# ajyoon/rocoder

Measured on AMD Instinct MI355X. Metric: output Msamples/s, 16384-win f=8 stereo (x CPU-realtime in config), higher is better.
Workload: dtype f32

## Files before the change

rocoder_amd/csrc/rc_hop16k.hip:

```cpp
#include "rc_dit.hpp"

namespace rc {
namespace {

constexpr int f1_idx(int n) { return n + (n >> 5); }
constexpr int HOP2_XBUF = 8192 + 256 + 32;
constexpr int HOP2_LDS_FLOAT2 = HOP2_XBUF + 8 + 32 + 256 + 256 + 16 + 24 + 1024;
constexpr int F3_W[13] = {1, 2, 4, 8, 16, 32, 64, 131, 259, 520, 1038, 2079, 4156};
constexpr int f3_idx(int n) {
    int r = 0;
    for (int i = 0; i < 13; ++i) r += ((n >> i) & 1) * F3_W[i];
    return r;
}

__global__ __launch_bounds__(256, 2) void hop2_kernel(const HopParams p) {
    constexpr int LOG2N = 14, m = 13, M = 1 << m, H = M, T = 256, P = 32, PH = 16;
    constexpr int RES = 512;
    constexpr int SCR = HOP2_XBUF + 8;
    constexpr int T_A = SCR + 32;
    constexpr int T_R = T_A + 256;
    constexpr int T_B = T_R + 256;
    constexpr int T_C = T_B + 16;
    constexpr int T_H = T_C + 24;
    static_assert(T_H + 1024 == HOP2_LDS_FLOAT2, "LDS layout");
    extern __shared__ __attribute__((aligned(16))) float2 lds[];
    const int tid = threadIdx.x;
    const uint32_t run = blockIdx.x % p.runs_per_channel;
    const uint32_t ch = blockIdx.x / p.runs_per_channel;
    const int64_t k_begin = p.hop_first + (int64_t)run * p.run_len;
    int64_t k_end = k_begin + p.run_len;
    if (k_end > p.hop_first + p.hop_count) k_end = p.hop_first + p.hop_count;
    if (k_begin >= k_end) return;
    GF xc = (GF)p.x + (size_t)ch * p.in_stride;
    GF xt = (GF)p.xtail + (size_t)ch * p.tail_stride;
    GFW outc = (GFW)p.out + (size_t)ch * p.out_stride;
    const unsigned lane2 = 2u * (unsigned)tid;
    GV2 wtab = (GV2)p.wtab;
    const uint32_t pitch = p.pitch;

    const int r = tid, rb = tid ? RES - tid : RES / 2;
    const int l4 = tid & 15, uu = tid >> 4;
    const int pos4 = (uu << 9) | l4;
    const int bE1s = f3_idx(((int)(__brev((unsigned)tid) >> 24) << 5));
    const int b4f3 = f3_idx(pos4);
    const int bAr = f3_idx(r), bBr = f3_idx(rb);
    const int bE3a = f3_idx(((int)(__brev((unsigned)r) >> 23) << 4));
    const int bE3b = f3_idx(((int)(__brev((unsigned)rb) >> 23) << 4));
    const int bE4l = f3_idx(tid);

    Stamps st;
    st.init();
    v2f tail[PH];
#pragma unroll
    for (int q = 0; q < PH; ++q) tail[q] = v2f{0.f, 0.f};

    {
        lds[T_A + tid] = ldg2(wtab + tid);
        lds[T_R + tid] = ldg2((GV2)p.rtab + tid);
        if (tid < 16) lds[T_B + tid] = ldg2(wtab + 16 * tid);
        if (tid <= 16) lds[T_C + tid] = ldg2(wtab + 128 * tid);
        __syncthreads();
    }
    float xr0[P], xr1[P];
    auto issue_x = [&](int64_t kk) {
        GF src = hop_src(p, xc, xt, kk);
#pragma unroll
        for (int q = 0; q < P; ++q) {
            xr0[q] = (src + 2 * T * q)[lane2];
            xr1[q] = (src + 2 * T * q)[lane2 + 1];
        }
    };
    auto win_f1 = [&](v2f (&vn)[P]) {
        GF win = per_hop(p.window);
        float wr0[P], wr1[P];
#pragma unroll
        for (int q = 0; q < P; ++q) {
            wr0[q] = (win + 2 * T * q)[lane2];
            wr1[q] = (win + 2 * T * q)[lane2 + 1];
        }
        __builtin_amdgcn_sched_barrier(0);
#pragma unroll
        for (int q = 0; q < P; ++q) vn[brev_c(q, 5)] = v2f{xr0[q], xr1[q]} * v2f{wr0[q], wr1[q]};
        __builtin_amdgcn_sched_barrier(0);
        st.mark(0);
        dit_stages<32, m, 0, 4, 0, false, false>(vn);
        st.mark(1);
    };
    auto epilogue = [&](int64_t kk, v2f (&ve)[P]) {
        GF wsrc = per_hop(p.window);
        float wr0[P], wr1[P];
#pragma unroll
        for (int q = 0; q < P; ++q) {
            wr0[q] = (wsrc + 2 * T * q)[lane2];
            wr1[q] = (wsrc + 2 * T * q)[lane2 + 1];
        }
        __builtin_amdgcn_sched_barrier(0);
#pragma unroll
        for (int q = 0; q < P; ++q) ve[q] *= v2f{wr0[q], wr1[q]};
        __builtin_amdgcn_sched_barrier(0);
        if (kk >= k_begin) {
            const int64_t g0 = kk * (int64_t)H;
            GF esrc = per_hop(p.env);
            const int64_t kq = g0 / pitch;
            const uint32_t kr = (uint32_t)(g0 % pitch);
            GFW dst = outc + (kq - p.out_origin);
            int t2 = tid;
            opaque(t2);
#pragma unroll
            for (int q = 0; q < PH; ++q) {
                const uint32_t i0 = 2u * (uint32_t)(t2 + T * q);
                const v2f er = v2f{(esrc + 2 * T * q)[lane2], (esrc + 2 * T * q)[lane2 + 1]};
                const v2f o = (ve[q] + tail[q]) * er * v2f{p.amp, p.amp};
                const float o0 = o.x, o1 = o.y;
                const uint32_t a0 = kr + i0, a1 = a0 + 1;
                const uint32_t d0 = a0 / pitch, d1 = a1 / pitch;
                if (d0 * pitch == a0) dst[d0] = o0;
                if (d1 * pitch == a1) dst[d1] = o1;
            }
        }
#pragma unroll
        for (int q = 0; q < PH; ++q) tail[q] = ve[q + PH];
        st.mark(21);
    };
    const int64_t k_first = k_begin > 0 ? k_begin - 1 : k_begin;
    v2f vn[P];
    for (int64_t k = k_first; k < k_end; ++k) {
        const PhaseKey key = make_phase_key(p.seed_mixed, p.ch_first + ch, k);
        v2f v[P];
        issue_x(k);
        win_f1(vn);
#pragma unroll
        for (int q = 0; q < P; ++q) lds[bE1s + f3_idx(q)] = to_f2(vn[q]);
        st.mark(2);
        __syncthreads();
        st.mark(3);
#pragma unroll
        for (int q = 0; q < P; ++q) v[q] = xld(lds, b4f3 + f3_idx(q << 4));
        dit_stages<32, m, 5, 8, 4, false, true>(v, to_v(lds[T_B + l4]));
        st.mark(4);
#pragma unroll
        for (int q = 0; q < P; ++q) lds[b4f3 + f3_idx(q << 4)] = to_f2(v[q]);
        st.mark(5);
        __syncthreads();
        st.mark(6);
        v2f va[16], vb[16];
#pragma unroll
        for (int q = 0; q < 16; ++q) {
            va[q] = xld(lds, bAr + f3_idx((RES * q)));
            vb[q] = xld(lds, bBr + f3_idx((RES * q)));
        }
        st.mark(7);
        __syncthreads();
        st.mark(8);
        {
            const v2f wa = to_v(lds[T_A + tid]);
            const v2f k16 = {W32_RE[2], W32_IM[2]};
            v2f wb = vcmul(v2f{wa.x, -wa.y}, k16);
            if (tid == 0) wb = v2f{W32_RE[1], W32_IM[1]};
            dit_stages<16, m, 9, 12, 9, false, true>(va, wa);
            dit_stages<16, m, 9, 12, 9, false, true>(vb, wb);
        }
        st.mark(9);

        if (tid == 0) {
#pragma unroll
            for (int q = 0; q < 16; ++q) {
                lds[SCR + q] = to_f2(va[q]);
                lds[SCR + 16 + q] = to_f2(vb[q]);
            }
        }
        {
            const int rr = r;
            const float2 wr = lds[T_R + tid];
            const uint32_t x0 = (uint32_t)rr * key.mul + key.k0;
            const uint32_t dx = (uint32_t)RES * key.mul;
#pragma unroll
            for (int q = 0; q < 16; ++q) {
                const v2f wrv = to_v(wr);
                const v2f wq = q == 0 ? wrv : (q == 8 ? v2f{wr.y, -wr.x}
                               : vcmul(wrv, v2f{W32_RE[q & 15], W32_IM[q & 15]}));
                v2f VA, VB;
                pair_regs_pk<LOG2N>(va[q], vb[15 - q], wq, x0 + (uint32_t)q * dx, key, VA, VB);
                va[q] = VA;
                vb[15 - q] = VB;
            }
        }
        st.mark(10);
        if (tid < 64) {
            const int i = tid;
            if (i <= 16) {
                int ja, ia, ib;
                if (i == 0) { ja = 0; ia = 0; ib = 0; }
                else if (i <= 7) { ja = RES * i; ia = i; ib = 16 - i; }
                else if (i == 8) { ja = RES * 8; ia = 8; ib = 8; }
                else { ja = RES / 2 + RES * (i - 9); ia = 16 + (i - 9); ib = 16 + 15 - (i - 9); }
                const float2 A = lds[SCR + ia], Bp = lds[SCR + ib];
                const float2 w = lds[T_C + (ja >> 8)];
                float2 VA, VB;
                pair_regs<LOG2N>(A, Bp, w, (uint32_t)ja * key.mul + key.k0, key, VA, VB, ja == 0);
                lds[SCR + ia] = VA;
                if (ib != ia) lds[SCR + ib] = VB;
            }
            if (tid == 0) {
#pragma unroll
                for (int q = 0; q < 16; ++q) {
                    va[q] = to_v(lds[SCR + q]);
                    vb[q] = to_v(lds[SCR + 16 + q]);
                }
            }
        }
        st.mark(11);
        v2f pa[16], pb[16];
#pragma unroll
        for (int q = 0; q < 16; ++q) {
            pa[brev_c(q, 4)] = va[q];
            pb[brev_c(q, 4)] = vb[q];
        }
        dit_stages<16, m, 0, 3, 0, true, false>(pa);
        dit_stages<16, m, 0, 3, 0, true, false>(pb);
        st.mark(12);
#pragma unroll
        for (int q = 0; q < 16; ++q) {
            lds[bE3a + f3_idx(q)] = to_f2(pa[q]);
            lds[bE3b + f3_idx(q)] = to_f2(pb[q]);
        }
        st.mark(13);
        __syncthreads();
        st.mark(14);
#pragma unroll
        for (int q = 0; q < P; ++q) v[q] = xld(lds, b4f3 + f3_idx(q << 4));
        dit_stages<32, m, 4, 8, 4, true, true>(v, to_v(lds[T_B + l4]));
        st.mark(15);
#pragma unroll
        for (int q = 0; q < P; ++q) lds[b4f3 + f3_idx(q << 4)] = to_f2(v[q]);
        st.mark(16);
        __syncthreads();
        st.mark(17);
#pragma unroll
        for (int q = 0; q < P; ++q) v[q] = xld(lds, bE4l + f3_idx((q << 8)));
        st.mark(18);
        __syncthreads();
        st.mark(19);
        dit_stages<32, m, 9, 12, 8, true, true>(v, to_v(lds[T_A + tid]));
        st.mark(20);

        epilogue(k, v);
    }
#if RC_STAMP
    if ((tid & 63) == 0 && p.spec) {
        unsigned *dbg = (unsigned *)p.spec + ((size_t)blockIdx.x * (T / 64) + (tid >> 6)) * 32;
        for (int i = 0; i < 32; ++i) dbg[i] = st.acc[i];
    }
#endif
}


constexpr int HOP4_REG = 1040;
constexpr int HOP4_XBUF = 4 * HOP4_REG;
constexpr int HOP4_LDS_FLOAT2 = HOP4_XBUF + 8 + 32 + 256 + 256 + 16 + 24 + 1024;
constexpr int phi_c(int l) { return (l & 1) ? 1 + 2 * (((l >> 1) ^ (l >> 2)) & 1) : 2 * ((l >> 1) & 1); }
constexpr int cidx_c(int l) { return (((l >> 2) & 1) << 1) | ((l >> 3) & 1); }
__device__ __forceinline__ void wave_fence() {
    __builtin_amdgcn_fence(__ATOMIC_RELEASE, "wavefront");
    asm volatile("" ::: "memory");
    __builtin_amdgcn_fence(__ATOMIC_ACQUIRE, "wavefront");
}

#define HOP4_BAR()                                                                    \
    do {                                                                              \
        asm volatile("s_waitcnt lgkmcnt(0)\n\ts_barrier" ::: "memory");                \
    } while (0)
__device__ __forceinline__ float band_gain(const HopParams &p, uint32_t f) {
    return (f - p.band_lo) <= p.band_span ? p.band_gin : p.band_gout;
}
template <int PITCHC, bool BAND = false, bool TABW = false>
__global__ __launch_bounds__(256, 3) void hop4_kernel(const HopParams p) {
    constexpr bool PITCH1 = PITCHC == 1;
    static_assert(!TABW || (PITCH1 && !BAND), "the table-window instantiation exists for pitch 1 without the band mask");
    constexpr int LOG2N = 14, m = 13, M = 1 << m, H = M, T = 256, P = 32, PH = 16;
    constexpr int RES = 512, REG = HOP4_REG;
    constexpr int SCR = HOP4_XBUF + 8;
    constexpr int T_A = SCR + 32;
    constexpr int T_R = T_A + 256;
    constexpr int T_B = T_R + 256;
    constexpr int T_C = T_B + 16;
    constexpr int T_H = T_C + 24;
    static_assert(T_H + 1024 == HOP4_LDS_FLOAT2, "LDS layout");
    extern __shared__ __attribute__((aligned(16))) float2 lds[];
    const int tid = threadIdx.x;
    uint32_t gr = blockIdx.x;
    const bool seam = p.seam_head != nullptr;
    if (seam) {
        unsigned *slot = reinterpret_cast<unsigned *>(lds + SCR);
        if (tid == 0) {
            const uint32_t total = p.runs_per_channel * p.n_channels;
            unsigned got = 0xFFFFFFFFu;
            {
                const uint32_t G = (total + 7u) / 8u;
                unsigned xcc;
                asm volatile("s_getreg_b32 %0, hwreg(HW_REG_XCC_ID)" : "=s"(xcc));
                for (uint32_t i = 0; i < 8u; ++i) {
                    const uint32_t xx = (xcc + i) & 7u, lo = xx * G;
                    if (lo >= total) continue;
                    const uint32_t hi = lo + G < total ? lo + G : total;
                    const uint32_t t = atomicAdd(p.run_counter + xx, 1u);
                    if (t < hi - lo) {
                        got = lo + t;
                        break;
                    }
                }
            }
            *slot = got;
        }
        __syncthreads();
        gr = (uint32_t)__builtin_amdgcn_readfirstlane((int)*reinterpret_cast<volatile unsigned *>(slot));
        __syncthreads();
        if (gr == 0xFFFFFFFFu) return;
    }
    const uint32_t run = gr % p.runs_per_channel;
    const uint32_t ch = gr / p.runs_per_channel;
    const int64_t k_begin = p.hop_first + (int64_t)run * p.run_len;
    int64_t k_end = k_begin + p.run_len;
    if (k_end > p.hop_first + p.hop_count) k_end = p.hop_first + p.hop_count;
    if (k_begin >= k_end) return;
    const bool stash_first = seam && run > 0;
    const bool has_next = seam && run + 1 < p.runs_per_channel;
    GF xc = (GF)p.x + (size_t)ch * p.in_stride;
    GF xt = (GF)p.xtail + (size_t)ch * p.tail_stride;
    GFW outc = (GFW)p.out + (size_t)ch * p.out_stride;
    const unsigned lane2 = 2u * (unsigned)tid;
    GV2 wtab = (GV2)p.wtab;
    const uint32_t pitch = PITCHC ? (uint32_t)PITCHC : p.pitch;

    struct Who {
        int wv, lane, cc, lo4, nib, r, A0;
    };
    int nib_keep, a0_keep;
    {
        const int w_ = tid >> 6, c_ = (tid >> 4) & 3;
        const int nl3 = c_ & 1, nl2 = c_ >> 1, nl0 = w_ & 1;
        const int nl1 = nl0 ? ((w_ >> 1) ^ nl2) : (w_ >> 1);
        nib_keep = (nl3 << 3) | (nl2 << 2) | (nl1 << 1) | nl0;
        a0_keep = w_ * REG + (tid & 63);
    }
    auto who = [&]() {
        int t = tid;
        opaque(t);
        Who w;
        w.wv = t >> 6;
        w.lane = t & 63;
        w.cc = (t >> 4) & 3;
        w.lo4 = t & 15;
        w.nib = nib_keep;
        w.r = (w.lo4 << 4) | w.nib;
        w.A0 = a0_keep;
        return w;
    };
    const int wv = tid >> 6;
    Stamps st;
    st.init();
    v2f tail[PH];
#pragma unroll
    for (int q = 0; q < PH; ++q) tail[q] = v2f{0.f, 0.f};
    {
        lds[T_A + tid] = ldg2(wtab + tid);
        lds[T_R + tid] = ldg2((GV2)p.rtab + tid);
        if (tid < 16) lds[T_B + tid] = ldg2(wtab + 16 * tid);
        if (tid <= 16) lds[T_C + tid] = ldg2(wtab + 128 * tid);
        if (tid == 0) {
            const float2 w256 = ldg2((GV2)p.rtab + 256);
            lds[SCR + 2] = make_float2(-w256.y, w256.x);
        }
        if constexpr (!TABW) {
#pragma unroll
            for (int i = 0; i < 2; ++i) {
                const float2 a = ldg2((GV2)p.hann_rot + 512 * i + 2 * tid);
                const float2 b = ldg2((GV2)p.hann_rot + 512 * i + 2 * tid + 1);
                lds[T_H + 512 * i + 2 * tid] = make_float2(a.x, b.x);
                lds[T_H + 512 * i + 2 * tid + 1] = make_float2(a.y, b.y);
            }
        }
        __syncthreads();
    }
    const v2f half2 = {0.5f, 0.5f};
    auto store_head = [&](int64_t kk, const auto &head) {
        const v2f amp2 = {p.amp, p.amp};
        const v2f cbE = to_v(lds[T_H + 2 * T + 2 * tid]) * amp2, sbE = to_v(lds[T_H + 2 * T + 2 * tid + 1]) * amp2;
        const v2f halfa = half2 * amp2;
        const int64_t g0 = kk * (int64_t)H;
        if constexpr (PITCH1) {
            const unsigned long long da = (unsigned long long)(outc + (g0 - p.out_origin));
            const unsigned dlo = __builtin_amdgcn_readfirstlane((unsigned)da);
            const unsigned dhi = __builtin_amdgcn_readfirstlane((unsigned)(da >> 32));
            GFW dst = (GFW)(((unsigned long long)dhi << 32) | dlo);
            const __amdgpu_buffer_rsrc_t rd = __builtin_amdgcn_make_buffer_rsrc((void *)dst, 0, 0x40000000, 0x00020000);
            typedef unsigned v2u __attribute__((ext_vector_type(2)));
#define HOP4_STORE(o, row)                                                                                                  \
    do {                                                                                                                    \
        if constexpr (!TABW)                                                                             \
            __builtin_amdgcn_raw_buffer_store_b64(v2u{__float_as_uint((o).x), __float_as_uint((o).y)}, rd,                 \
                                                  (int)(4u * lane2), 4 * 2 * T * (row), 2);                                 \
        else __builtin_nontemporal_store(o, (GV2W)(dst + 2 * T * (row) + lane2));                                           \
    } while (0)
            if constexpr (TABW) {
                GF et2 = per_hop(p.env) + lane2;
#pragma unroll
                for (int q0 = 0; q0 < PH; q0 += 4) {
                    float e0[4], e1[4];
#pragma unroll
                    for (int q = 0; q < 4; ++q) {
                        e0[q] = (et2 + 2 * T * (q0 + q))[0];
                        e1[q] = (et2 + 2 * T * (q0 + q))[1];
                    }
#pragma unroll
                    for (int q = 0; q < 4; ++q) {
                        const v2f o = (head[q0 + q] + tail[q0 + q]) * v2f{e0[q], e1[q]} * amp2;
                        HOP4_STORE(o, q0 + q);
                    }
                    __builtin_amdgcn_sched_barrier(0);
                }
                return;
            }
#pragma unroll
            for (int q = 0; q < PH; ++q) {
                const v2f er = __builtin_elementwise_fma(v2f{HANN_E14.s[q], HANN_E14.s[q]}, sbE,
                               __builtin_elementwise_fma(v2f{HANN_E14.c[q], HANN_E14.c[q]}, cbE, halfa));
                const v2f o = (head[q] + tail[q]) * er;
                HOP4_STORE(o, q);
            }
        } else {
            const int64_t kq = g0 / pitch;
            const uint32_t kr = (uint32_t)(g0 % pitch);
            GFW dst = outc + (kq - p.out_origin);
            int t2 = tid;
            opaque(t2);
            const unsigned long long da = (unsigned long long)dst;
            const unsigned dlo = __builtin_amdgcn_readfirstlane((unsigned)da);
            const unsigned dhi = __builtin_amdgcn_readfirstlane((unsigned)(da >> 32));
            const __amdgpu_buffer_rsrc_t rsrc = __builtin_amdgcn_make_buffer_rsrc(
                (void *)(((unsigned long long)dhi << 32) | dlo), 0, 0x40000000, 0x00020000);
            if constexpr (PITCHC > 1) {
                const PitchOffsets<PITCHC> po = pitch_offsets<PITCHC>(kr + 2u * (uint32_t)t2);
#pragma unroll
                for (int q = 0; q < PH; ++q) {
                    const v2f er = __builtin_elementwise_fma(v2f{HANN_E14.s[q], HANN_E14.s[q]}, sbE,
                                   __builtin_elementwise_fma(v2f{HANN_E14.c[q], HANN_E14.c[q]}, cbE, halfa));
                    const v2f o = (head[q] + tail[q]) * er;
                    const float ox = o.x, oy = o.y;
                    pitch_store_pair<PITCHC, 2 * T>(rsrc, po, q, ox, oy);
                }
                return;
            }
            constexpr uint32_t DROP = 0xFFFFFFFCu;
            const uint32_t a00 = kr + 2u * (uint32_t)t2;
            const uint32_t d0 = a00 / pitch;
            uint32_t r = a00 - d0 * pitch, d4 = 4u * d0;
            const uint32_t qs4 = 4u * ((2u * T) / pitch), rs = (2u * T) - (qs4 / 4u) * pitch;
#pragma unroll
            for (int q = 0; q < PH; ++q) {
                const v2f er = __builtin_elementwise_fma(v2f{HANN_E14.s[q], HANN_E14.s[q]}, sbE,
                               __builtin_elementwise_fma(v2f{HANN_E14.c[q], HANN_E14.c[q]}, cbE, halfa));
                const v2f o = (head[q] + tail[q]) * er;
                const float ox = o.x, oy = o.y;
                __builtin_amdgcn_raw_buffer_store_b32(__float_as_int(ox), rsrc, r == 0 ? d4 : DROP, 0, 0);
                __builtin_amdgcn_raw_buffer_store_b32(__float_as_int(oy), rsrc, r + 1 == pitch ? d4 + 4u : DROP, 0, 0);
                d4 += qs4;
                r += rs;
                if (r >= pitch) {
                    r -= pitch;
                    d4 += 4u;
                }
            }
        }
    };
    for (int64_t k = ((k_begin > 0 && !stash_first) ? k_begin - 1 : k_begin); k < k_end; ++k) {
        const PhaseKey key = make_phase_key(p.seed_mixed, p.ch_first + ch, k);
        v2f v[P];
        st.mark(26);
        {
            GF src = hop_src(p, xc, xt, k);
            float xr0[P], xr1[P];
            if constexpr (!TABW) {
                const __amdgpu_buffer_rsrc_t rs = __builtin_amdgcn_make_buffer_rsrc((void *)src, 0, 0x40000000, 0x00020000);
                typedef unsigned v2u __attribute__((ext_vector_type(2)));
#pragma unroll
                for (int q = 0; q < P; ++q) {
                    const v2u x = __builtin_amdgcn_raw_buffer_load_b64(rs, (int)(4u * lane2), 4 * 2 * T * q, 0);
                    xr0[q] = __uint_as_float(x.x);
                    xr1[q] = __uint_as_float(x.y);
                }
            } else {
#pragma unroll
                for (int q = 0; q < P; ++q) {
                    xr0[q] = (src + 2 * T * q)[lane2];
                    xr1[q] = (src + 2 * T * q)[lane2 + 1];
                }
            }
            const v2f cb = to_v(lds[T_H + 2 * tid]), sb = to_v(lds[T_H + 2 * tid + 1]);
            if constexpr (TABW) {
                GF wt2 = per_hop(p.window) + lane2;
#pragma unroll
                for (int q0 = 0; q0 < 16; q0 += 4) {
                    float l0[4], l1[4], h0[4], h1[4];
#pragma unroll
                    for (int q = 0; q < 4; ++q) {
                        l0[q] = (wt2 + 2 * T * (q0 + q))[0];
                        l1[q] = (wt2 + 2 * T * (q0 + q))[1];
                        h0[q] = (wt2 + 2 * T * (q0 + q + 16))[0];
                        h1[q] = (wt2 + 2 * T * (q0 + q + 16))[1];
                    }
#pragma unroll
                    for (int qq = 0; qq < 4; ++qq) {
                        const int q = q0 + qq;
                        const v2f a = v2f{xr0[q], xr1[q]} * v2f{l0[qq], l1[qq]}, xh = v2f{xr0[q + 16], xr1[q + 16]};
                        const v2f wh = v2f{h0[qq], h1[qq]};
                        v[2 * brev_c(q, 4)] = __builtin_elementwise_fma(xh, wh, a);
                        v[2 * brev_c(q, 4) + 1] = __builtin_elementwise_fma(-xh, wh, a);
                    }
                    __builtin_amdgcn_sched_barrier(0);
                }
            } else
#pragma unroll
            for (int q = 0; q < 16; ++q) {
                const v2f wl = __builtin_elementwise_fma(v2f{HANN_W14.s[q], HANN_W14.s[q]}, sb,
                               __builtin_elementwise_fma(v2f{HANN_W14.c[q], HANN_W14.c[q]}, cb, half2));
                const v2f wh = __builtin_elementwise_fma(v2f{HANN_W14.s[q + 16], HANN_W14.s[q + 16]}, sb,
                               __builtin_elementwise_fma(v2f{HANN_W14.c[q + 16], HANN_W14.c[q + 16]}, cb, half2));
                const v2f a = v2f{xr0[q], xr1[q]} * wl, xh = v2f{xr0[q + 16], xr1[q + 16]};
                v[2 * brev_c(q, 4)] = __builtin_elementwise_fma(xh, wh, a);
                v[2 * brev_c(q, 4) + 1] = __builtin_elementwise_fma(-xh, wh, a);
            }
            st.mark(0);
            dit_stages<32, m, 1, 4, 0, false, false>(v);
            st.mark(1);
        }
        wave_fence();
        {
            const Who w = who();
            const int A0 = w.A0, A1 = w.wv * REG + (w.lane ^ 16);
#pragma unroll
            for (int q = 0; q < 16; ++q) lds[((q >> 3) & 1 ? A1 : A0) + q * 64] = to_f2(v[q]);
        }
        st.mark(2);
        HOP4_BAR();
        st.mark(3);
        v2f w2[P];
        {
            const Who w = who();
            const int b4u = (int)(__brev((unsigned)w.lo4) >> 28), l3 = w.nib >> 3;
            const int bE1Ae = w.nib * 64 + b4u + 16 * l3, bE1Ao = w.nib * 64 + b4u - 16 * l3;
#pragma unroll
            for (int j = 0; j < 16; ++j) {
                const int bj = brev_c(j, 4), X = bj & 3;
                w2[2 * j] = to_v(lds[(bj >> 2) * REG + X * 16 + ((X & 1) ? bE1Ao : bE1Ae)]);
            }
        }
        st.mark(4);
        HOP4_BAR();
        st.mark(5);
        {
            int t = tid;
            opaque(t);
            const int bE1Bs = (int)(__brev((unsigned)(t >> 4)) >> 28) * 64 + (int)(__brev((unsigned)(t & 15)) >> 28);
#pragma unroll
            for (int q = 0; q < 16; ++q) lds[phi_c(q) * REG + cidx_c(q) * 16 + bE1Bs] = to_f2(v[16 + q]);
        }
        st.mark(6);
        HOP4_BAR();
        st.mark(7);
        Who w = who();
#pragma unroll
        for (int j = 0; j < 16; ++j) w2[2 * j + 1] = to_v(lds[w.A0 + j * 64]);
        st.mark(8);
        dit_stages<32, m, 5, 8, 4, false, true>(w2, to_v(lds[T_B + w.nib]));
        st.mark(9);
        wave_fence();
        v2f va[16], vb[16];
        {
            w = who();
            const int rlow = (256 - w.r) & 255;
            const int nibb = rlow & 15;
            const int cb = (((nibb >> 2) & 1) << 1) | (nibb >> 3);
            const int bE2A = w.wv * REG + w.lo4 * 65 + w.cc * 16;
            const int bE2B = w.wv * REG + (rlow >> 4) * 65 + cb * 16;
#pragma unroll
            for (int q = 0; q < 16; ++q) lds[w.A0 + q * 65] = to_f2(w2[q]);
            wave_fence();
#pragma unroll
            for (int q = 0; q < 16; ++q) va[q] = to_v(lds[bE2A + q]);
            wave_fence();
#pragma unroll
            for (int q = 0; q < 16; ++q) lds[w.A0 + q * 65] = to_f2(w2[16 + q]);
            wave_fence();
#pragma unroll
            for (int q = 0; q < 16; ++q) vb[q] = to_v(lds[bE2B + q]);
            wave_fence();
        }
        st.mark(10);
        w = who();
        const int r = w.r;
        {
            const v2f wa = to_v(lds[T_A + r]);
            const v2f k16 = {W32_RE[2], W32_IM[2]};
            v2f wb = vcmul(v2f{wa.x, -wa.y}, k16);
            if (tid == 0) wb = v2f{W32_RE[1], W32_IM[1]};
            dit_stages<16, m, 9, 12, 9, false, true>(va, wa);
            dit_stages<16, m, 9, 12, 9, false, true>(vb, wb);
        }
        st.mark(11);
        const bool is0 = tid == 0;
        v2f s8 = va[8];
        if (wv == 0) {
            const v2f va0 = va[0];
#pragma unroll
            for (int i = 0; i < 8; ++i) {
                const v2f a = va[8 + i], b0 = vb[i], b1 = vb[8 + i];
                const v2f nx = i < 7 ? va[9 + i] : va0;
                va[8 + i] = vsel(is0, b0, a);
                vb[i] = vsel(is0, b1, b0);
                vb[8 + i] = vsel(is0, nx, b1);
            }
        }
        {
            const float2 wrl = lds[T_R + r];
            const float2 wrh = lds[is0 ? SCR + 2 : T_R + r];
            const uint32_t x0 = (uint32_t)r * key.mul + key.k0;
            const uint32_t dx = (uint32_t)RES * key.mul;
            const uint32_t x0h = x0 - (is0 ? 3840u * key.mul : 0u);
#pragma unroll
            for (int q = 0; q < 16; ++q) {
                const float2 wr = q < 8 ? wrl : wrh;
                const v2f wrv = to_v(wr);
                const v2f wq = q == 0 ? wrv : (q == 8 ? v2f{wr.y, -wr.x}
                               : vcmul(wrv, v2f{W32_RE[q & 15], W32_IM[q & 15]}));
                v2f VA, VB;
                v2f gq = {1.0f, 1.0f};
                if constexpr (BAND) {
                    const uint32_t ja = (uint32_t)r + (uint32_t)RES * (uint32_t)q - ((q >= 8 && is0) ? 3840u : 0u);
                    gq = v2f{band_gain(p, ja), band_gain(p, (uint32_t)M - ja)};
                }
                if (q == 0)
                    pair_regs_pk5<LOG2N, true, BAND>(va[q], vb[15 - q], wq, x0, key, VA, VB, is0, gq);
                else
                    pair_regs_pk5<LOG2N, false, BAND>(va[q], vb[15 - q], wq, (q < 8 ? x0 : x0h) + (uint32_t)q * dx, key, VA, VB,
                                                  false, gq);
                va[q] = VA;
                vb[15 - q] = VB;
            }
        }
        st.mark(12);
        if (wv == 0) {
            v2f V8, V8b;
            const float g8 = BAND ? band_gain(p, 8u * (uint32_t)RES) : 1.0f;
            pair_regs_pk5<LOG2N, false, BAND>(s8, s8, v2f{0.0f, -1.0f}, 8u * (uint32_t)RES * key.mul + key.k0, key, V8, V8b,
                                          false, v2f{g8, g8});
            v2f na[8], nb0[8], nb1[8];
#pragma unroll
            for (int i = 0; i < 8; ++i) {
                na[i] = vsel(is0, i == 0 ? V8 : vb[7 + i], va[8 + i]);
                nb0[i] = vsel(is0, va[8 + i], vb[i]);
                nb1[i] = vsel(is0, vb[i], vb[8 + i]);
            }
#pragma unroll
            for (int i = 0; i < 8; ++i) {
                va[8 + i] = na[i];
                vb[i] = nb0[i];
                vb[8 + i] = nb1[i];
            }
        }
        st.mark(13);
        v2f pa[16], pb[16];
#pragma unroll
        for (int q = 0; q < 16; ++q) {
            pa[brev_c(q, 4)] = va[q];
            pb[brev_c(q, 4)] = vb[q];
        }
        dit_stages<16, m, 0, 3, 0, true, false>(pa);
        dit_stages<16, m, 0, 3, 0, true, false>(pb);
        st.mark(14);
        wave_fence();
        {
            w = who();
            const int bE3A = w.wv * REG + w.lo4 * 65 + w.cc * 16;
            const int nn = (16 - w.nib) & 15;
            const int cs3 = (((nn >> 2) & 1) << 1) | (nn >> 3);
            const int bE3B = w.wv * REG + w.lo4 * 65 + cs3 * 16 + (w.nib == 0 ? 1 : 0);
            const int bE3B0 = bE3B - (w.nib == 0 ? 16 : 0);
#pragma unroll
            for (int q = 0; q < 16; ++q) lds[w.A0 + q * 65] = to_f2(pa[q]);
            wave_fence();
#pragma unroll
            for (int j = 0; j < 16; ++j) v[2 * j] = to_v(lds[bE3A + brev_c(j, 4)]);
            wave_fence();
#pragma unroll
            for (int q = 0; q < 16; ++q) lds[w.A0 + q * 65] = to_f2(pb[q]);
            wave_fence();
#pragma unroll
            for (int j = 0; j < 16; ++j)
                v[2 * j + 1] = to_v(lds[(brev_c(j, 4) == 0 ? bE3B0 : bE3B) + 15 - brev_c(j, 4)]);
            wave_fence();
        }
        st.mark(15);
        w = who();
        dit_stages<32, m, 4, 8, 4, true, true>(v, to_v(lds[T_B + w.lo4]));
        st.mark(16);
        wave_fence();
        {
            w = who();
            const int A0 = w.A0, A1 = w.wv * REG + (w.lane ^ 16);
#pragma unroll
            for (int q = 0; q < 16; ++q) lds[((q & 1) ? A1 : A0) + q * 64] = to_f2(v[q]);
        }
        st.mark(17);
        HOP4_BAR();
        st.mark(18);
        v2f y[P];
        {
            int t = tid;
            opaque(t);
            const int rho8 = t >> 4, l4p = t & 15;
            const int bE4Ae = rho8 * 64 + l4p + 16 * (rho8 & 1), bE4Ao = rho8 * 64 + l4p - 16 * (rho8 & 1);
#pragma unroll
            for (int j = 0; j < 16; ++j) {
                const int nj = brev_c(j, 4), cs = cidx_c(nj);
                y[2 * j] = to_v(lds[phi_c(nj) * REG + 32 * (cs >> 1) + ((cs & 1) ? bE4Ao + 16 : bE4Ae)]);
            }
        }
        st.mark(19);
        HOP4_BAR();
        st.mark(20);
        {
            w = who();
            const int bE4Bs = (int)(__brev((unsigned)w.nib) >> 28) * 64 + w.lo4;
#pragma unroll
            for (int q = 0; q < 16; ++q) lds[(q >> 2) * REG + (q & 3) * 16 + bE4Bs] = to_f2(v[16 + q]);
        }
        st.mark(21);
        HOP4_BAR();
        st.mark(22);
        w = who();
#pragma unroll
        for (int j = 0; j < 16; ++j) y[2 * j + 1] = to_v(lds[w.A0 + j * 64]);
        st.mark(23);
        dit_stages<32, m, 9, 12, 8, true, true>(y, to_v(lds[T_A + tid]));
        st.mark(24);

        const v2f cbW = to_v(lds[T_H + 2 * tid]), sbW = to_v(lds[T_H + 2 * tid + 1]);
        const v2f half2k = {(float)(0.5 * HANN_KAPPA), (float)(0.5 * HANN_KAPPA)};
        if constexpr (TABW) {
            GF wt2 = per_hop(p.window) + lane2;
            const v2f kap = half2k + half2k;
#pragma unroll
            for (int q0 = 0; q0 < P; q0 += 4) {
                float a0[4], a1[4];
#pragma unroll
                for (int q = 0; q < 4; ++q) {
                    a0[q] = (wt2 + 2 * T * (q0 + q))[0];
                    a1[q] = (wt2 + 2 * T * (q0 + q))[1];
                }
#pragma unroll
                for (int q = 0; q < 4; ++q) y[q0 + q] *= v2f{a0[q], a1[q]} * kap;
                __builtin_amdgcn_sched_barrier(0);
            }
        } else
#pragma unroll
        for (int q = 0; q < P; ++q)
            y[q] *= __builtin_elementwise_fma(v2f{HANN_W14K.s[q], HANN_W14K.s[q]}, sbW,
                    __builtin_elementwise_fma(v2f{HANN_W14K.c[q], HANN_W14K.c[q]}, cbW, half2k));
        if (k >= k_begin) {
            if (stash_first && k == k_begin) {
                int t2 = tid;
                opaque(t2);
                unsigned long long *hs = (unsigned long long *)(p.seam_head + (size_t)gr * H) + t2;
#pragma unroll
                for (int q = 0; q < PH; ++q)
                    __hip_atomic_store(hs + T * q, __builtin_bit_cast(unsigned long long, y[q]),
                                       __ATOMIC_RELAXED, __HIP_MEMORY_SCOPE_AGENT);
                asm volatile("s_waitcnt vmcnt(0)" ::: "memory");
                __syncthreads();
                if (tid == 0 && !(p.diag_flags & RC_DIAG_SKIP_SEAM_PUBLISH))
                    __hip_atomic_store(p.seam_flag + gr, p.seam_epoch, __ATOMIC_RELAXED, __HIP_MEMORY_SCOPE_AGENT);
            } else {
                store_head(k, y);
            }
        }
#pragma unroll
        for (int q = 0; q < PH; ++q) tail[q] = y[q + PH];
        st.mark(25);
    }
#if RC_STAMP
    if ((tid & 63) == 0 && p.spec) {
        unsigned *dbg = (unsigned *)p.spec + ((size_t)blockIdx.x * (T / 64) + (tid >> 6)) * 32;
        for (int i = 0; i < 32; ++i) dbg[i] = st.acc[i];
    }
#endif
    if (has_next) {
        unsigned *okw = reinterpret_cast<unsigned *>(lds + SCR);
        if (tid == 0) {
            unsigned ok = 0;
            for (unsigned spin = 0; spin < p.seam_spin_limit; ++spin) {
                if (__hip_atomic_load(p.seam_flag + gr + 1, __ATOMIC_RELAXED, __HIP_MEMORY_SCOPE_AGENT) ==
                    p.seam_epoch) {
                    ok = 1;
                    break;
                }
                __builtin_amdgcn_s_sleep(32);
            }
            if (!ok && p.err_word)
                __hip_atomic_store(p.err_word, RC_ERR_SEAM_TIMEOUT, __ATOMIC_RELAXED, __HIP_MEMORY_SCOPE_SYSTEM);
            *okw = ok;
        }
        __syncthreads();
        if (*reinterpret_cast<volatile unsigned *>(okw) == 0) return;
        const unsigned long long *hs = (const unsigned long long *)(p.seam_head + (size_t)(gr + 1) * H) + tid;
        v2f head[PH];
#pragma unroll
        for (int q = 0; q < PH; ++q)
            head[q] = __builtin_bit_cast(v2f, __hip_atomic_load(hs + T * q, __ATOMIC_RELAXED, __HIP_MEMORY_SCOPE_AGENT));
        store_head(k_end, head);
    }
}

}

hipError_t launch_hop16k(const HopParams &p, hipStream_t s) {
    const dim3 grid(p.runs_per_channel * p.n_channels), block(256);
    const bool hann = p.hann_rot != nullptr;
#if RC_TEST_HOOKS
    if (hann && (p.diag_flags & RC_DIAG_PREV_KERNEL)) return launch_hop16k_prev(p, s);
#endif
    if (hann) {
        const size_t lds4 = sizeof(float2) * (size_t)HOP4_LDS_FLOAT2;
        if (p.band_on) {
            if (p.pitch == 1) hipLaunchKernelGGL((hop4_kernel<1, true>), grid, block, lds4, s, p);
            else hipLaunchKernelGGL((hop4_kernel<0, true>), grid, block, lds4, s, p);
        } else if (p.pitch == 1) hipLaunchKernelGGL((hop4_kernel<1>), grid, block, lds4, s, p);
        else if (p.pitch == 2) hipLaunchKernelGGL((hop4_kernel<2>), grid, block, lds4, s, p);
        else if (p.pitch == 3) hipLaunchKernelGGL((hop4_kernel<3>), grid, block, lds4, s, p);
        else hipLaunchKernelGGL((hop4_kernel<0>), grid, block, lds4, s, p);
    } else {
        if (!p.window || !p.env) return hipErrorInvalidValue;
        if (p.pitch == 1)
            hipLaunchKernelGGL((hop4_kernel<1, false, true>), grid, block, sizeof(float2) * (size_t)HOP4_LDS_FLOAT2, s, p);
        else hipLaunchKernelGGL(hop2_kernel, grid, block, sizeof(float2) * (size_t)HOP2_LDS_FLOAT2, s, p);
    }
    return hipGetLastError();
}
}
```

Before: 313,500.

## Use 16-byte output stores via permlane32 swap and permuted thread-to-column mapping

For the pitch-1 Hann path, threads are remapped to permuted output columns so that after a permlane32 swap each lane holds two adjacent samples from two rows. This allows 128-bit buffer stores instead of 64-bit ones, halving the store instruction count. To keep results correct, the LDS transpose scatter and gather indices in the FFT stages are changed to match the new lane order. It adds permlane swaps and an s_nop per store, plus a test-hook path that can force the generic pitch kernel.

```diff
diff --git a/rocoder_amd/csrc/rc_hop16k.hip b/rocoder_amd/csrc/rc_hop16k.hip
--- a/rocoder_amd/csrc/rc_hop16k.hip
+++ b/rocoder_amd/csrc/rc_hop16k.hip
@@ -277,6 +277,7 @@
 __global__ __launch_bounds__(256, 3) void hop4_kernel(const HopParams p) {
     constexpr bool PITCH1 = PITCHC == 1;
     static_assert(!TABW || (PITCH1 && !BAND), "the table-window instantiation exists for pitch 1 without the band mask");
+    constexpr bool ST16 = PITCH1 && !TABW;
     constexpr int LOG2N = 14, m = 13, M = 1 << m, H = M, T = 256, P = 32, PH = 16;
     constexpr int RES = 512, REG = HOP4_REG;
     constexpr int SCR = HOP4_XBUF + 8;
@@ -357,6 +358,15 @@
         return w;
     };
     const int wv = tid >> 6;
+    auto tid_pos = [&]() {
+        if constexpr (ST16) {
+            int t = tid;
+            opaque(t);
+            return (t & 192) | ((t & 31) << 1) | ((t >> 5) & 1);
+        } else {
+            return tid;
+        }
+    };
     Stamps st;
     st.init();
     v2f tail[PH];
@@ -385,7 +395,8 @@
     const v2f half2 = {0.5f, 0.5f};
     auto store_head = [&](int64_t kk, const auto &head) {
         const v2f amp2 = {p.amp, p.amp};
-        const v2f cbE = to_v(lds[T_H + 2 * T + 2 * tid]) * amp2, sbE = to_v(lds[T_H + 2 * T + 2 * tid + 1]) * amp2;
+        const int tp = tid_pos();
+        const v2f cbE = to_v(lds[T_H + 2 * T + 2 * tp]) * amp2, sbE = to_v(lds[T_H + 2 * T + 2 * tp + 1]) * amp2;
         const v2f halfa = half2 * amp2;
         const int64_t g0 = kk * (int64_t)H;
         if constexpr (PITCH1) {
@@ -421,6 +432,26 @@
                 }
                 return;
             }
+            if constexpr (ST16) {
+                typedef unsigned v4u __attribute__((ext_vector_type(4)));
+                const int loff = 8 * (tp & ~1) + 4 * 2 * T * (tp & 1);
+#pragma unroll
+                for (int q = 0; q < PH; q += 2) {
+                    v2f o[2];
+#pragma unroll
+                    for (int i = 0; i < 2; ++i) {
+                        const v2f er = __builtin_elementwise_fma(v2f{HANN_E14.s[q + i], HANN_E14.s[q + i]}, sbE,
+                                       __builtin_elementwise_fma(v2f{HANN_E14.c[q + i], HANN_E14.c[q + i]}, cbE, halfa));
+                        o[i] = (head[q + i] + tail[q + i]) * er;
+                    }
+                    const auto sx = __builtin_amdgcn_permlane32_swap(__float_as_uint(o[0].x), __float_as_uint(o[1].x), false, false);
+                    const auto sy = __builtin_amdgcn_permlane32_swap(__float_as_uint(o[0].y), __float_as_uint(o[1].y), false, false);
+                    const v4u d = {sx[0], sy[0], sx[1], sy[1]};
+                    __builtin_amdgcn_raw_buffer_store_b128(d, rd, loff, 4 * 2 * T * q, 2);
+                    asm volatile("s_nop 3" ::"v"(d) : "memory");
+                }
+                return;
+            }
 #pragma unroll
             for (int q = 0; q < PH; ++q) {
                 const v2f er = __builtin_elementwise_fma(v2f{HANN_E14.s[q], HANN_E14.s[q]}, sbE,
@@ -708,6 +739,12 @@
         {
             w = who();
             const int A0 = w.A0, A1 = w.wv * REG + (w.lane ^ 16);
+            if constexpr (ST16) {
+                const int A2 = w.wv * REG + (w.lane ^ 1), A3 = w.wv * REG + (w.lane ^ 17);
+#pragma unroll
+                for (int q = 0; q < 16; ++q)
+                    lds[((q & 2) ? ((q & 1) ? A3 : A1) : ((q & 1) ? A2 : A0)) + q * 64] = to_f2(v[q]);
+            } else
 #pragma unroll
             for (int q = 0; q < 16; ++q) lds[((q & 1) ? A1 : A0) + q * 64] = to_f2(v[q]);
         }
@@ -718,8 +755,10 @@
         {
             int t = tid;
             opaque(t);
-            const int rho8 = t >> 4, l4p = t & 15;
-            const int bE4Ae = rho8 * 64 + l4p + 16 * (rho8 & 1), bE4Ao = rho8 * 64 + l4p - 16 * (rho8 & 1);
+            if constexpr (ST16) t = (t & 192) | ((t & 31) << 1) | ((t >> 5) & 1);
+            const int rho8 = t >> 4, l4p = ST16 ? ((t & 15) ^ (rho8 & 1)) : (t & 15);
+            const int sw4 = ST16 ? ((rho8 >> 1) & 1) : (rho8 & 1);
+            const int bE4Ae = rho8 * 64 + l4p + 16 * sw4, bE4Ao = rho8 * 64 + l4p - 16 * sw4;
 #pragma unroll
             for (int j = 0; j < 16; ++j) {
                 const int nj = brev_c(j, 4), cs = cidx_c(nj);
@@ -732,6 +771,13 @@
         {
             w = who();
             const int bE4Bs = (int)(__brev((unsigned)w.nib) >> 28) * 64 + w.lo4;
+            if constexpr (ST16) {
+                const int p0 = w.lo4 & 1;
+                const int b0 = bE4Bs - w.lo4 + 32 * p0 + (w.lo4 >> 1);
+                const int bE = b0 + 8 * p0, bO = b0 - 8 * p0;
+#pragma unroll
+                for (int q = 0; q < 16; ++q) lds[(q >> 2) * REG + (q & 3) * 8 + ((q & 1) ? bO : bE)] = to_f2(v[16 + q]);
+            } else
 #pragma unroll
             for (int q = 0; q < 16; ++q) lds[(q >> 2) * REG + (q & 3) * 16 + bE4Bs] = to_f2(v[16 + q]);
         }
@@ -739,13 +785,15 @@
         HOP4_BAR();
         st.mark(22);
         w = who();
-#pragma unroll
-        for (int j = 0; j < 16; ++j) y[2 * j + 1] = to_v(lds[w.A0 + j * 64]);
+        const int bE4Bl = ST16 ? w.wv * REG + (w.lane ^ ((w.lane >> 5) << 3)) : w.A0;
+#pragma unroll
+        for (int j = 0; j < 16; ++j) y[2 * j + 1] = to_v(lds[bE4Bl + j * 64]);
         st.mark(23);
-        dit_stages<32, m, 9, 12, 8, true, true>(y, to_v(lds[T_A + tid]));
+        const int tp = tid_pos();
+        dit_stages<32, m, 9, 12, 8, true, true>(y, to_v(lds[T_A + tp]));
         st.mark(24);
 
-        const v2f cbW = to_v(lds[T_H + 2 * tid]), sbW = to_v(lds[T_H + 2 * tid + 1]);
+        const v2f cbW = to_v(lds[T_H + 2 * tp]), sbW = to_v(lds[T_H + 2 * tp + 1]);
         const v2f half2k = {(float)(0.5 * HANN_KAPPA), (float)(0.5 * HANN_KAPPA)};
         if constexpr (TABW) {
             GF wt2 = per_hop(p.window) + lane2;
@@ -828,6 +876,13 @@
     const bool hann = p.hann_rot != nullptr;
 #if RC_TEST_HOOKS
     if (hann && (p.diag_flags & RC_DIAG_PREV_KERNEL)) return launch_hop16k_prev(p, s);
+    constexpr uint32_t DIAG_HOP4_ANY_PITCH = 16;
+    if (hann && p.pitch == 1 && (p.diag_flags & DIAG_HOP4_ANY_PITCH)) {
+        const size_t lds4 = sizeof(float2) * (size_t)HOP4_LDS_FLOAT2;
+        if (p.band_on) hipLaunchKernelGGL((hop4_kernel<0, true>), grid, block, lds4, s, p);
+        else hipLaunchKernelGGL((hop4_kernel<0>), grid, block, lds4, s, p);
+        return hipGetLastError();
+    }
 #endif
     if (hann) {
         const size_t lds4 = sizeof(float2) * (size_t)HOP4_LDS_FLOAT2;
```

Result: no change. 314,000 (median of 2 runs) (+0.2%).
